# dedis/kyber

Measured on AMD Instinct MI355X. Metric: scalar-muls/s + pairings/s per node; MSM sec at 2^20 points, higher is better.
Workload: dtype int32 limbs (radix 2^25.5), int64 accumulate; 1 GPU; Ed25519 batched fixed-base + var-base scalar-mul, 2^20 scalars per GPU (BASELINE.json configs[1]); elements_per_gpu=1048576

## Files before the change

kyber_amd/csrc/context.h:

```cpp
#pragma once
#include <hip/hip_runtime.h>
#include <stddef.h>
#include <stdint.h>

#include <stdlib.h>
#include <string.h>

#include <algorithm>
#include <condition_variable>
#include <initializer_list>
#include <map>
#include <mutex>
#include <string>
#include <vector>
#include <utility>

#include "../../include/kyber_hip.h"
#include "hd.h"

namespace kyb {

void set_error(const std::string& msg);

#define KYB_HIP_CHECK(expr)                                                              \
    do {                                                                                 \
        hipError_t e_ = (expr);                                                          \
        if (e_ != hipSuccess) {                                                          \
            ::kyb::set_error(std::string(#expr) + ": " + hipGetErrorString(e_));         \
            return KYB_E_HIP;                                                            \
        }                                                                                \
    } while (0)

struct DeviceCtx {
    int device = -1;
    int num_cu = 0;
    bool ready = false;
    std::mutex mu;
    std::recursive_mutex enq_mu;
    int32_t* ed_base_tab = nullptr;
    int32_t* ed_wide_tab = nullptr;
    int64_t ed_wide_build_us = 0;
    struct StreamBuf {
        void* p = nullptr;
        size_t cap = 0;
    };
    std::map<std::pair<int, hipStream_t>, StreamBuf> sws;
    static constexpr int NSTAGE = 12, NPOOL = 2, NPIN = 6;
    struct StagePool {
        bool busy = false;
        hipStream_t stream = nullptr;
        void* stage[NSTAGE] = {};
        size_t stage_cap[NSTAGE] = {};
        hipStream_t pipe[3] = {};
        void* pin_in[NPIN] = {};
        void* pin_out[NPIN] = {};
        bool pinned = false;
    };
    StagePool pools[NPOOL];
    std::mutex stage_mu;
    std::condition_variable stage_cv;
    std::map<std::pair<int, hipStream_t>, std::string> fb_hint;
};
constexpr size_t PIN_SLOT_ELEMS = size_t(1) << 17;
constexpr size_t PIN_IN_BYTES = PIN_SLOT_ELEMS * 64, PIN_OUT_BYTES = PIN_SLOT_ELEMS * 33;
int ctx_pin_slots(DeviceCtx::StagePool* pool);
void par_memcpy(void* dst, const void* src, size_t bytes);

inline int check_flags(uint32_t flags, int npoint, bool point_out, const char* who) {
    const uint32_t allowed = KYB_F_UNCOMPRESSED | (point_out ? KYB_F_UNCOMPRESSED_OUT : 0u) | (((1u << npoint) - 1u) << 8);
    if (flags & ~allowed) {
        set_error(std::string(who) + ": unknown or inapplicable flag bits");
        return KYB_E_ARG;
    }
    return KYB_OK;
}

inline int make_dst(DstArg& d, const uint8_t* dst, size_t dst_len, const char* who) {
    if (dst_len > 255 || (dst_len && !dst)) {
        set_error(std::string(who) + ": the domain separation tag must be at most 255 bytes");
        return KYB_E_ARG;
    }
    memset(&d, 0, sizeof d);
    if (dst_len) memcpy(d.b, dst, dst_len);
    d.len = (uint32_t)dst_len;
    return KYB_OK;
}

int md_count();
size_t md_threshold();
void shard_range(size_t n, int rank, int world, size_t* lo, size_t* hi);
std::vector<int> md_devices();
int md_run_impl(size_t n, int (*thunk)(void*, int, size_t, size_t), void* arg, const std::vector<int>* on = nullptr);
template <class F>
int md_run(size_t n, F&& f, const std::vector<int>* on = nullptr) {
    return md_run_impl(n, [](void* a, int s, size_t lo, size_t hi) -> int { return (*static_cast<F*>(a))(s, lo, hi); }, &f, on);
}
inline bool md_active(size_t n) { return md_count() > 1 && n >= md_threshold() && n >= (size_t)md_count(); }

int get_ctx(DeviceCtx** out);
int ctx_workspace(DeviceCtx* ctx, int kind, hipStream_t stream, size_t bytes, void** out, bool* grew = nullptr);

inline void fb_hint_set(DeviceCtx* ctx, int kind, hipStream_t stream, const std::string* key) {
    std::lock_guard<std::mutex> lk(ctx->mu);
    if (key) ctx->fb_hint[std::make_pair(kind, stream)] = *key;
    else ctx->fb_hint.erase(std::make_pair(kind, stream));
}
inline bool fb_hint_is(DeviceCtx* ctx, int kind, hipStream_t stream, const std::string& key) {
    std::lock_guard<std::mutex> lk(ctx->mu);
    auto it = ctx->fb_hint.find(std::make_pair(kind, stream));
    return it != ctx->fb_hint.end() && it->second == key;
}

struct StageScope {
    DeviceCtx* ctx;
    DeviceCtx::StagePool* pool = nullptr;
    int next = 0;
    explicit StageScope(DeviceCtx* c) : ctx(c) {
        static const int npool = [] {
            const char* e = getenv("KYB_STAGE_POOLS");
            const int v = e ? atoi(e) : 0;
            return v >= 1 && v <= DeviceCtx::NPOOL ? v : DeviceCtx::NPOOL;
        }();
        {
            std::unique_lock<std::mutex> lk(c->stage_mu);
            for (;;) {
                for (int i = 0; i < npool && !pool; i++)
                    if (!c->pools[i].busy) pool = &c->pools[i];
                if (pool) break;
                c->stage_cv.wait(lk);
            }
            pool->busy = true;
        }
        if (!pool->stream && hipStreamCreateWithFlags(&pool->stream, hipStreamDefault) != hipSuccess) pool->stream = nullptr;
        current() = this;
    }
    ~StageScope() {
        current() = nullptr;
        {
            std::lock_guard<std::mutex> lk(ctx->stage_mu);
            pool->busy = false;
        }
        ctx->stage_cv.notify_one();
    }
    StageScope(const StageScope&) = delete;
    StageScope& operator=(const StageScope&) = delete;
    hipStream_t stream() const { return pool->stream; }
    static StageScope*& current() {
        static thread_local StageScope* cur = nullptr;
        return cur;
    }
};
struct StageBuf {
    void* p = nullptr;
    static int too_many() {
        set_error("staging: no scope / too many buffers");
        return KYB_E_ARG;
    }
    int alloc(size_t bytes) {
        StageScope* sc = StageScope::current();
        if (!sc || sc->next >= DeviceCtx::NSTAGE) return too_many();
        const int slot = sc->next++;
        DeviceCtx::StagePool* c = sc->pool;
        if (c->stage_cap[slot] < bytes || !c->stage[slot]) {
            if (c->stage[slot]) {
                hipFree(c->stage[slot]);
                c->stage[slot] = nullptr;
                c->stage_cap[slot] = 0;
            }
            const size_t cap = bytes + bytes / 4 + 256;
            if (hipMalloc(&c->stage[slot], cap) != hipSuccess) {
                set_error("hipMalloc failed");
                return KYB_E_ALLOC;
            }
            c->stage_cap[slot] = cap;
        }
        p = c->stage[slot];
        return KYB_OK;
    }
    static constexpr size_t BOUNCE_MIN = size_t(4) << 20;
    int upload(const void* src, size_t bytes) {
        int rc = alloc(bytes);
        if (rc) return rc;
        if (!bytes) return KYB_OK;
        if (bytes < BOUNCE_MIN) {
            const hipStream_t st = StageScope::current()->stream();
            KYB_HIP_CHECK(hipMemcpyAsync(p, src, bytes, hipMemcpyHostToDevice, st));
            KYB_HIP_CHECK(hipStreamSynchronize(st));
            return KYB_OK;
        }
        return bounce(const_cast<void*>(src), bytes, true);
    }
    int download(void* dst, size_t bytes) {
        if (!bytes) return KYB_OK;
        if (bytes < BOUNCE_MIN) {
            const hipStream_t st = StageScope::current()->stream();
            KYB_HIP_CHECK(hipMemcpyAsync(dst, p, bytes, hipMemcpyDeviceToHost, st));
            KYB_HIP_CHECK(hipStreamSynchronize(st));
            return KYB_OK;
        }
        return bounce(dst, bytes, false);
    }
    int bounce(void* host, size_t bytes, bool up) {
        StageScope* sc = StageScope::current();
        DeviceCtx::StagePool* c = sc->pool;
        const hipStream_t st = sc->stream();
        int rc = ctx_pin_slots(c);
        if (rc) return rc;
        hipEvent_t ev[2];
        for (int k = 0; k < 2; k++) KYB_HIP_CHECK(hipEventCreateWithFlags(&ev[k], hipEventDisableTiming));
        const size_t piece = PIN_IN_BYTES;
        const size_t npiece = (bytes + piece - 1) / piece;
        rc = KYB_OK;
        for (size_t i = 0; i <= npiece && rc == KYB_OK; i++) {
            if (up) {
                if (i == npiece) break;
                const size_t off = i * piece, len = std::min(piece, bytes - off);
                if (i >= 2 && hipEventSynchronize(ev[i & 1]) != hipSuccess) rc = KYB_E_HIP;
                par_memcpy(c->pin_in[i & 1], (const uint8_t*)host + off, len);
                if (hipMemcpyAsync((uint8_t*)p + off, c->pin_in[i & 1], len, hipMemcpyHostToDevice, st) != hipSuccess ||
                    hipEventRecord(ev[i & 1], st) != hipSuccess)
                    rc = KYB_E_HIP;
            } else {
                if (i < npiece) {
                    const size_t off = i * piece, len = std::min(piece, bytes - off);
                    if (hipMemcpyAsync(c->pin_in[i & 1], (const uint8_t*)p + off, len, hipMemcpyDeviceToHost, st) != hipSuccess ||
                        hipEventRecord(ev[i & 1], st) != hipSuccess)
                        rc = KYB_E_HIP;
                }
                if (i >= 1 && rc == KYB_OK) {
                    const size_t off = (i - 1) * piece, len = std::min(piece, bytes - off);
                    if (hipEventSynchronize(ev[(i - 1) & 1]) != hipSuccess) rc = KYB_E_HIP;
                    else par_memcpy((uint8_t*)host + off, c->pin_in[(i - 1) & 1], len);
                }
            }
        }
        if (hipStreamSynchronize(st) != hipSuccess) rc = KYB_E_HIP;
        for (int k = 0; k < 2; k++) hipEventDestroy(ev[k]);
        if (rc == KYB_E_HIP) set_error("staging: page-locked bounce copy failed");
        return rc;
    }
};

struct HostIn {
    const void* p;
    size_t bytes;
    bool absent = false;
};
struct HostOut {
    void* p;
    size_t bytes;
    size_t slack = 0;
};
template <class F>
int staged_call(DeviceCtx* ctx, std::initializer_list<HostIn> in, std::initializer_list<HostOut> out, F&& run) {
    if (in.size() > (size_t)DeviceCtx::NSTAGE || out.size() > (size_t)DeviceCtx::NSTAGE) return StageBuf::too_many();
    StageScope sc(ctx);
    void* d_in[DeviceCtx::NSTAGE] = {};
    void* d_out[DeviceCtx::NSTAGE] = {};
    StageBuf b;
    int k = 0;
    for (const HostIn& h : in) {
        b.p = nullptr;
        if (!h.absent)
            if (int rc = b.upload(h.p, h.bytes)) return rc;
        d_in[k++] = b.p;
    }
    k = 0;
    for (const HostOut& h : out) {
        if (int rc = b.alloc(h.bytes + h.slack)) return rc;
        d_out[k++] = b.p;
    }
    if (int rc = run(d_in, d_out, sc.stream())) return rc;
    k = 0;
    for (const HostOut& h : out) {
        b.p = d_out[k++];
        if (h.p)
            if (int rc = b.download(h.p, h.bytes)) return rc;
    }
    return KYB_OK;
}

int ed25519_build_tables(DeviceCtx* ctx);
void ed25519_free_tables(DeviceCtx* ctx);

}
```

kyber_amd/csrc/ed25519.hip:

```cpp
#ifndef KYB_TU_WAVES
#define KYB_TU_WAVES 2
#endif
#include "context.h"
#include "ed25519_dev.cuh"
#include "ed25519_launch.h"
#include "msm.cuh"
#include "ed25519_h2c.cuh"
#include <stdlib.h>
#include <string.h>

#include <algorithm>
#include <atomic>
#include <chrono>
#include <thread>
#include <vector>

namespace kyb {


template <int G = 2>
__global__ void ed25519_build_base_table_kernel(int32_t* __restrict__ tab, const uint32_t* __restrict__ point,
                                                uint32_t* __restrict__ ok, int rows = ED_TAB_POS * ED_TAB_ENT) {
    const int t = blockIdx.x * blockDim.x + threadIdx.x;
    if (t >= rows) return;
    ge_p3 B;
    if (point) {
        uint32_t pw[8];
        load_words8(pw, point);
        const bool good = ge_p3_fromwords(B, pw);
        if (t == 0) *ok = good ? 1u : 0u;
    } else {
        B.X = fe_bx(); B.Y = fe_by(); fe_1(B.Z); B.T = fe_bt();
    }
    ed_comb_row<G>(tab + (size_t)t * ED_TAB_STRIDE, t, B);
}

__global__ __launch_bounds__(ED_ENC_BLOCK, KYB_TU_WAVES) void ed25519_encode_kernel(size_t n, const int32_t* __restrict__ proj,
                                                            const uint8_t* __restrict__ status,
                                                            uint32_t* __restrict__ out) {
    __shared__ int32_t pre_lds[EncPreLds<ED_ENC_BLOCK>::WORDS];
    static_assert(ED_ENC_BLOCK % 64 == 0 && sizeof(pre_lds) <= 80 * 1024 && sizeof(pre_lds) / (ED_ENC_BLOCK / 64) * 4 <= 160 * 1024,
                  "LDS: at least two blocks on a CU, and a wave on every SIMD");
    EncPreLds<ED_ENC_BLOCK> pre{pre_lds + threadIdx.x};
    ed_encode_chunk(n, proj, ed_encode_first(), blockDim.x, pre, [&](size_t i, uint32_t (&w)[8]) {
        if (status && status[i]) {
#pragma unroll
            for (int k = 0; k < 8; k++) w[k] = 0;
        }
        store_words8(out + i * 8, w);
    });
}


template <int G>
__global__ __launch_bounds__(256, 3) void ed25519_mul_base_kernel(
    size_t n, const uint32_t* __restrict__ scalars, uint32_t* __restrict__ out,
    const int32_t* __restrict__ tab, uint32_t flags, int32_t* __restrict__ proj) {
    const bool full = (flags & KYB_F_VARTIME) != 0;
    for (size_t idx = (size_t)blockIdx.x * blockDim.x + threadIdx.x; idx < n;
         idx += (size_t)gridDim.x * blockDim.x) {
        uint32_t a[8];
        load_words8(a, scalars + idx * 8);
        int8_t e[65];
        recode16(e, a, full);
        ge_p3 h;
        ge_p3_0(h);
        ge_precomp t;
        ge_p1p1 r;
        const int npos = full ? EdComb<G>::POS : EdComb<G>::POS_CT;
        EdCombDigits<G> digits(e);
#pragma unroll 1
        for (int k = 0; k < npos; k++) {
            const int d = digits.next(k);
            if (full && __ballot(d != 0) == 0) continue;
            select_precomp_tab<EdComb<G>::ENT>(t, tab, k, d);
            ge_madd(r, h, t);
            ge_p1p1_to_p3(h, r);
        }
        if (proj) {
            store_proj(proj, idx, h);
            continue;
        }
        uint32_t w[8];
        ge_p3_towords(w, h);
        store_words8(out + idx * 8, w);
    }
}

KYB_DEV void select_precomp_uniform(ge_precomp& t, const int32_t* __restrict__ tab, int i, int b) {
    const bool neg = b < 0;
    const int babs = neg ? -b : b;
    const int pos = i >> 1, mult = (i & 1) ? 16 : 1;
    fe_1(t.ypx);
    fe_1(t.ymx);
    fe_0(t.xy2d);
#pragma unroll 1
    for (int m = 1; m <= 8; m++) {
        const int4* e = reinterpret_cast<const int4*>(tab + (size_t)(pos * ED_TAB_ENT + (m * mult - 1)) * ED_TAB_STRIDE);
        int32_t w[32];
#pragma unroll
        for (int q = 0; q < 8; q++) {
            const int4 x = e[q];
            w[4 * q] = x.x;
            w[4 * q + 1] = x.y;
            w[4 * q + 2] = x.z;
            w[4 * q + 3] = x.w;
        }
        const int32_t keep = -(int32_t)(babs == m);
#pragma unroll
        for (int l = 0; l < 10; l++) {
            t.ypx.v[l] ^= (t.ypx.v[l] ^ w[l]) & keep;
            t.ymx.v[l] ^= (t.ymx.v[l] ^ w[10 + l]) & keep;
            t.xy2d.v[l] ^= (t.xy2d.v[l] ^ w[20 + l]) & keep;
        }
    }
    ge_precomp_cneg(t, neg);
}
__global__ __launch_bounds__(256, 3) void ed25519_mul_base_uniform_kernel(
    size_t n, const uint32_t* __restrict__ scalars, uint32_t* __restrict__ out,
    const int32_t* __restrict__ tab, int32_t* __restrict__ proj) {
    for (size_t idx = (size_t)blockIdx.x * blockDim.x + threadIdx.x; idx < n;
         idx += (size_t)gridDim.x * blockDim.x) {
        uint32_t a[8];
        load_words8(a, scalars + idx * 8);
        int8_t e[65];
        recode16(e, a, false);
        ge_p3 h;
        ge_p3_0(h);
        ge_precomp t;
        ge_p1p1 r;
        EdCombDigits<1> digits(e);
#pragma unroll 1
        for (int i = 0; i < 64; i++) {
            select_precomp_uniform(t, tab, i, digits.next(i));
            ge_madd(r, h, t);
            ge_p1p1_to_p3(h, r);
        }
        if (proj) {
            store_proj(proj, idx, h);
            continue;
        }
        uint32_t w[8];
        ge_p3_towords(w, h);
        store_words8(out + idx * 8, w);
    }
}


template <bool GTAB, bool UNI = false>
__global__ __launch_bounds__(128, 3) void ed25519_mul_kernel(
    size_t n, const uint32_t* __restrict__ scalars, const uint32_t* __restrict__ points,
    size_t points_stride, uint32_t* __restrict__ out, uint8_t* __restrict__ status,
    uint32_t flags, int32_t* __restrict__ proj, int4* __restrict__ gtab) {
    const size_t idx = (size_t)blockIdx.x * blockDim.x + threadIdx.x;
    if (idx >= n) return;
    const bool full = !UNI && (flags & KYB_F_VARTIME) != 0;
    uint32_t pw[8], a[8];
    load_words8(pw, points + idx * points_stride);
    load_words8(a, scalars + idx * 8);
    ge29_p3 A;
    const bool ok = ge_p3_fromwords(A, pw);
    int8_t e[65];
    recode16(e, a, full);
    ge29_p3 h;
    const int vt_top = full ? wave_top_digit(a) : 63;
    if constexpr (GTAB) {
        TabGlobal_t<fe29> tab{gtab + idx * 80};
        ge_scalarmult_w4<UNI, true>(h, e, A, full, tab, vt_top);
    } else {
        TabScratch_t<fe29> tab;
        ge_scalarmult_w4<UNI, true>(h, e, A, full, tab, vt_top);
    }
    if (proj) {
        store_proj(proj, idx, h);
        if (status) status[idx] = ok ? KYB_ST_OK : KYB_ST_BAD_POINT;
        return;
    }
    uint32_t w[8];
    ge_p3_towords(w, h);
    if (!ok) {
#pragma unroll
        for (int i = 0; i < 8; i++) w[i] = 0;
    }
    store_words8(out + idx * 8, w);
    if (status) status[idx] = ok ? KYB_ST_OK : KYB_ST_BAD_POINT;
}

int ed25519_build_tables(DeviceCtx* ctx) {
    KYB_HIP_CHECK(hipMalloc(&ctx->ed_base_tab, ED_TAB_WORDS * sizeof(int32_t)));
    hipLaunchKernelGGL(ed25519_build_base_table_kernel<2>, dim3((ED_TAB_POS * ED_TAB_ENT + 63) / 64), dim3(64), 0,
                       nullptr, ctx->ed_base_tab, (const uint32_t*)nullptr, (uint32_t*)nullptr, ED_TAB_POS * ED_TAB_ENT);
    KYB_HIP_CHECK(hipGetLastError());
    const auto t0 = std::chrono::steady_clock::now();
    KYB_HIP_CHECK(hipMalloc(&ctx->ed_wide_tab, ED_WIDE_WORDS * sizeof(int32_t)));
    hipLaunchKernelGGL(ed25519_build_base_table_kernel<ED_COMB_G>, dim3((EdWide::ROWS + 63) / 64), dim3(64), 0, nullptr,
                       ctx->ed_wide_tab, (const uint32_t*)nullptr, (uint32_t*)nullptr, EdWide::ROWS);
    KYB_HIP_CHECK(hipGetLastError());
    KYB_HIP_CHECK(hipStreamSynchronize(nullptr));
    ctx->ed_wide_build_us = std::chrono::duration_cast<std::chrono::microseconds>(std::chrono::steady_clock::now() - t0).count();
    return KYB_OK;
}
void ed25519_free_tables(DeviceCtx* ctx) {
    if (ctx->ed_base_tab) hipFree(ctx->ed_base_tab);
    if (ctx->ed_wide_tab) hipFree(ctx->ed_wide_tab);
    ctx->ed_base_tab = ctx->ed_wide_tab = nullptr;
}

constexpr size_t ENC_DEFER_MIN = 4096;


static int launch_mul_base(DeviceCtx* ctx, size_t n, const void* d_scalars, void* d_out, uint32_t flags,
                           hipStream_t st, const int32_t* tab = nullptr) {
    const bool wide = !tab && !(flags & KYB_F_UNIFORM);
    if (!tab) tab = wide ? ctx->ed_wide_tab : ctx->ed_base_tab;
    if (n == 0) return KYB_OK;
    const int block = 256;
    size_t want = (n + block - 1) / block;
    size_t cap = (size_t)ctx->num_cu * 8;
    int grid = (int)(want < cap ? want : cap);
    EdSlab w{};
    std::lock_guard<std::recursive_mutex> enq_lock(ctx->enq_mu);
    if (n >= ENC_DEFER_MIN)
        if (int rc = ed_slab(ctx, st, ED_SLAB_MUL_BASE, n, &w)) return rc;
    if (flags & KYB_F_UNIFORM) {
        hipLaunchKernelGGL(ed25519_mul_base_uniform_kernel, dim3(grid), dim3(block), 0, st, n,
                           (const uint32_t*)d_scalars, (uint32_t*)d_out, tab, w.proj);
    } else {
        const auto kernel = wide ? ed25519_mul_base_kernel<ED_COMB_G> : ed25519_mul_base_kernel<2>;
        hipLaunchKernelGGL(kernel, dim3(grid), dim3(block), 0, st, n, (const uint32_t*)d_scalars, (uint32_t*)d_out, tab,
                           flags, w.proj);
    }
    if (w.proj)
        hipLaunchKernelGGL(ed25519_encode_kernel, ed_encode_grid(n), dim3(ED_ENC_BLOCK), 0, st, n, w.proj,
                           (const uint8_t*)nullptr, (uint32_t*)d_out);
    KYB_HIP_CHECK(hipGetLastError());
    return KYB_OK;
}
static int launch_mul(size_t n, const void* d_scalars, const void* d_points, size_t stride, void* d_out,
                      void* d_status, uint32_t flags, hipStream_t st) {
    if (n == 0) return KYB_OK;
    const int block = 128;
    size_t grid = (n + block - 1) / block;
    EdSlab w{};
    uint8_t* stat = (uint8_t*)d_status;
    DeviceCtx* ctx;
    int rc = get_ctx(&ctx);
    if (rc) return rc;
    std::lock_guard<std::recursive_mutex> enq_lock(ctx->enq_mu);
    const bool defer = n >= ENC_DEFER_MIN, uni = (flags & KYB_F_UNIFORM) != 0;
    const auto kernel = defer ? (uni ? ed25519_mul_kernel<true, true> : ed25519_mul_kernel<true, false>)
                              : (uni ? ed25519_mul_kernel<false, true> : ed25519_mul_kernel<false, false>);
    if (defer) {
        if ((rc = ed_slab(ctx, st, ed_slab_mul(stat == nullptr), n, &w))) return rc;
        if (!stat) stat = w.status;
    }
    hipLaunchKernelGGL(kernel, dim3((unsigned)grid), dim3(block), 0, st, n, (const uint32_t*)d_scalars,
                       (const uint32_t*)d_points, stride, (uint32_t*)d_out, stat, flags, w.proj, w.gtab);
    if (w.proj)
        hipLaunchKernelGGL(ed25519_encode_kernel, ed_encode_grid(n), dim3(ED_ENC_BLOCK), 0, st, n, w.proj,
                           (const uint8_t*)stat, (uint32_t*)d_out);
    KYB_HIP_CHECK(hipGetLastError());
    return KYB_OK;
}

}

using namespace kyb;

static bool ed_mul_flags_bad(uint32_t flags) {
    return (flags & ~(KYB_F_VARTIME | KYB_F_UNIFORM)) || (flags & (KYB_F_VARTIME | KYB_F_UNIFORM)) == (KYB_F_VARTIME | KYB_F_UNIFORM);
}

extern "C" {

int kyb_ed25519_mul_base_dev(size_t n, const void* d_scalars, void* d_out, uint32_t flags, void* stream) {
    if ((n && (!d_scalars || !d_out)) || ed_mul_flags_bad(flags)) {
        set_error("kyb_ed25519_mul_base_dev: bad argument");
        return KYB_E_ARG;
    }
    DeviceCtx* ctx;
    int rc = get_ctx(&ctx);
    if (rc) return rc;
    return launch_mul_base(ctx, n, d_scalars, d_out, flags, (hipStream_t)stream);
}

int kyb_ed25519_mul_dev(size_t n, const void* d_scalars, const void* d_points, void* d_out, void* d_status,
                        uint32_t flags, void* stream) {
    if ((n && (!d_scalars || !d_points || !d_out)) || ed_mul_flags_bad(flags)) {
        set_error("kyb_ed25519_mul_dev: bad argument");
        return KYB_E_ARG;
    }
    DeviceCtx* ctx;
    int rc = get_ctx(&ctx);
    if (rc) return rc;
    return launch_mul(n, d_scalars, d_points, 8, d_out, d_status, flags, (hipStream_t)stream);
}

static int mul_host(size_t n, const uint8_t* scalars, const uint8_t* points, size_t stride, uint8_t* out,
                    uint8_t* status, uint32_t flags);

int kyb_ed25519_mul_base(size_t n, const uint8_t* scalars, uint8_t* out, uint32_t flags) {
    if ((n && (!scalars || !out)) || ed_mul_flags_bad(flags)) {
        set_error("kyb_ed25519_mul_base: bad argument");
        return KYB_E_ARG;
    }
    if (n == 0) return KYB_OK;
    if (md_active(n))
        return md_run(n, [&](int, size_t lo, size_t hi) { return kyb_ed25519_mul_base(hi - lo, scalars + 32 * lo, out + 32 * lo, flags); });
    return mul_host(n, scalars, nullptr, 0, out, nullptr, flags);
}

constexpr size_t PIPE_CHUNK_MAX = PIN_SLOT_ELEMS;
constexpr int PIPE_SLOTS = DeviceCtx::NPIN, PIPE_STREAMS = 3;
static size_t pipe_chunk(const DeviceCtx* ctx) {
    if (const char* e = getenv("KYB_PIPE_CHUNK")) {
        const size_t v = (size_t)strtoull(e, nullptr, 10) & ~size_t(63);
        if (v >= 4096) return std::min(PIPE_CHUNK_MAX, v);
    }
    (void)ctx;
    return size_t(1) << 17;
}
static int pipe_nstreams() {
    if (const char* e = getenv("KYB_PIPE_STREAMS")) {
        const int v = atoi(e);
        if (v >= 1 && v <= PIPE_STREAMS) return v;
    }
    return 2;
}
constexpr size_t SAME_BASE_TABLE_MIN = 16384;

static int pipe_streams(DeviceCtx::StagePool* pool) {
    for (int i = 0; i < PIPE_STREAMS; i++)
        if (!pool->pipe[i]) KYB_HIP_CHECK(hipStreamCreateWithFlags(&pool->pipe[i], hipStreamNonBlocking));
    return KYB_OK;
}

static int mul_host(size_t n, const uint8_t* scalars, const uint8_t* points, size_t stride, uint8_t* out,
                    uint8_t* status, uint32_t flags) {
    DeviceCtx* ctx;
    int rc = get_ctx(&ctx);
    if (rc) return rc;
    bool fixed = points == nullptr;
    const size_t npts = fixed ? 0 : (stride ? n : 1);
    StageScope sc_(ctx);
    StageBuf d_s, d_p, d_o, d_st, d_tab;
    if ((rc = d_s.alloc(n * 32))) return rc;
    if ((rc = d_p.alloc(npts * 32))) return rc;
    if ((rc = d_o.alloc(n * 32))) return rc;
    if ((rc = d_st.alloc(n))) return rc;
    const int32_t* tab = nullptr;
    if (!fixed && !stride && (n >= SAME_BASE_TABLE_MIN || (flags & KYB_F_UNIFORM))) {
        if ((rc = d_tab.alloc(ED_TAB_WORDS * sizeof(int32_t) + 256))) return rc;
        uint32_t* d_ok = (uint32_t*)((uint8_t*)d_tab.p + ED_TAB_WORDS * sizeof(int32_t));
        KYB_HIP_CHECK(hipMemcpy(d_p.p, points, 32, hipMemcpyHostToDevice));
        hipLaunchKernelGGL(ed25519_build_base_table_kernel<2>, dim3((ED_TAB_POS * ED_TAB_ENT + 63) / 64), dim3(64), 0, sc_.stream(),
                           (int32_t*)d_tab.p, (const uint32_t*)d_p.p, d_ok, ED_TAB_POS * ED_TAB_ENT);
        uint32_t ok = 0;
        KYB_HIP_CHECK(hipMemcpy(&ok, d_ok, 4, hipMemcpyDeviceToHost));
        if (!ok) {
            memset(out, 0, n * 32);
            if (status) memset(status, KYB_ST_BAD_POINT, n);
            return KYB_OK;
        }
        if (status) memset(status, 0, n);
        tab = (const int32_t*)d_tab.p;
        fixed = true;
    }
    auto launch = [&](size_t off, size_t cnt, hipStream_t st) -> int {
        uint8_t* s = (uint8_t*)d_s.p + off * 32;
        uint8_t* o = (uint8_t*)d_o.p + off * 32;
        if (fixed) return launch_mul_base(ctx, cnt, s, o, flags, st, tab);
        const uint8_t* p = (const uint8_t*)d_p.p + (stride ? off * 32 : 0);
        return launch_mul(cnt, s, p, stride, o, (uint8_t*)d_st.p + off, flags, st);
    };
    const size_t PIPE_CHUNK = pipe_chunk(ctx);
    if (n < 2 * PIPE_CHUNK) {
        KYB_HIP_CHECK(hipMemcpy(d_s.p, scalars, n * 32, hipMemcpyHostToDevice));
        if (npts) KYB_HIP_CHECK(hipMemcpy(d_p.p, points, npts * 32, hipMemcpyHostToDevice));
        if ((rc = launch(0, n, nullptr))) return rc;
        if ((rc = d_o.download(out, n * 32))) return rc;
        if (status && !fixed) rc = d_st.download(status, n);
        return rc;
    }
    DeviceCtx::StagePool* pool = sc_.pool;
    if ((rc = pipe_streams(pool))) return rc;
    const int nstreams = pipe_nstreams();
    const bool per_point = !fixed && stride;
    const bool want_status = status && !fixed;
    if ((rc = ctx_pin_slots(pool))) return rc;
    const size_t nchunks = (n + PIPE_CHUNK - 1) / PIPE_CHUNK;
    std::vector<hipEvent_t> ev_out(nchunks);
    for (size_t i = 0; i < nchunks; i++) KYB_HIP_CHECK(hipEventCreateWithFlags(&ev_out[i], hipEventDisableTiming));
    auto enqueue = [&](size_t i) -> int {
        const size_t off = i * PIPE_CHUNK, cnt = std::min(PIPE_CHUNK, n - off);
        uint8_t* pin = (uint8_t*)pool->pin_in[i % PIPE_SLOTS];
        uint8_t* pout = (uint8_t*)pool->pin_out[i % PIPE_SLOTS];
        hipStream_t s_k = pool->pipe[i % nstreams];
        par_memcpy(pin, scalars + off * 32, cnt * 32);
        if (per_point) par_memcpy(pin + PIPE_CHUNK_MAX * 32, points + off * 32, cnt * 32);
        int r;
        if (fixed) {
            r = launch_mul_base(ctx, cnt, pin, pout, flags, s_k, tab);
        } else {
            const uint8_t* p = per_point ? pin + PIPE_CHUNK_MAX * 32 : (const uint8_t*)d_p.p;
            r = launch_mul(cnt, pin, p, stride, pout, (uint8_t*)d_st.p + off, flags, s_k);
        }
        if (r) return r;
        if (want_status)
            KYB_HIP_CHECK(hipMemcpyAsync(pout + PIPE_CHUNK_MAX * 32, (uint8_t*)d_st.p + off, cnt, hipMemcpyDeviceToHost, s_k));
        KYB_HIP_CHECK(hipEventRecord(ev_out[i], s_k));
        return KYB_OK;
    };
    auto drain = [&](size_t i) -> int {
        const size_t off = i * PIPE_CHUNK, cnt = std::min(PIPE_CHUNK, n - off);
        KYB_HIP_CHECK(hipEventSynchronize(ev_out[i]));
        const uint8_t* pout = (const uint8_t*)pool->pin_out[i % PIPE_SLOTS];
        par_memcpy(out + off * 32, pout, cnt * 32);
        if (want_status) memcpy(status + off, pout + PIPE_CHUNK_MAX * 32, cnt);
        return KYB_OK;
    };
    if (!fixed && !stride) KYB_HIP_CHECK(hipMemcpy(d_p.p, points, 32, hipMemcpyHostToDevice));
    std::atomic<size_t> enqueued{0}, drained{0};
    std::atomic<int> drain_rc{KYB_OK};
    std::atomic<bool> stop{false};
    const int device = ctx->device;
    std::string drain_err;
    std::thread drainer([&] {
        if (hipSetDevice(device) != hipSuccess) {
            drain_err = "ed25519 host pipeline: hipSetDevice failed on the drain thread";
            drain_rc.store(KYB_E_HIP);
            return;
        }
        for (size_t i = 0; i < nchunks; i++) {
            while (enqueued.load(std::memory_order_acquire) <= i) {
                if (stop.load(std::memory_order_acquire)) return;
                std::this_thread::yield();
            }
            const int r = drain(i);
            if (r) {
                drain_err = kyb_last_error();
                drain_rc.store(r);
                return;
            }
            drained.store(i + 1, std::memory_order_release);
        }
    });
    for (size_t i = 0; i < nchunks && rc == KYB_OK; i++) {
        while (i >= (size_t)PIPE_SLOTS && drained.load(std::memory_order_acquire) + PIPE_SLOTS <= i && drain_rc.load() == KYB_OK)
            std::this_thread::yield();
        if (drain_rc.load() != KYB_OK) break;
        rc = enqueue(i);
        if (rc == KYB_OK) enqueued.store(i + 1, std::memory_order_release);
    }
    if (rc != KYB_OK) stop.store(true, std::memory_order_release);
    drainer.join();
    if (rc == KYB_OK && (rc = drain_rc.load()) != KYB_OK) set_error(drain_err);
    hipError_t e2 = hipSuccess;
    for (int i = 0; i < PIPE_STREAMS; i++) {
        const hipError_t e = hipStreamSynchronize(pool->pipe[i]);
        if (e != hipSuccess) e2 = e;
    }
    for (size_t i = 0; i < nchunks; i++) hipEventDestroy(ev_out[i]);
    if (rc == KYB_OK && e2 != hipSuccess) {
        set_error("ed25519 host pipeline: stream synchronisation failed");
        rc = KYB_E_HIP;
    }
    return rc;
}

int kyb_ed25519_mul(size_t n, const uint8_t* scalars, const uint8_t* points, uint8_t* out, uint8_t* status,
                    uint32_t flags) {
    if ((n && (!scalars || !points || !out)) || ed_mul_flags_bad(flags)) {
        set_error("kyb_ed25519_mul: bad argument");
        return KYB_E_ARG;
    }
    if (n == 0) return KYB_OK;
    if (md_active(n))
        return md_run(n, [&](int, size_t lo, size_t hi) {
            return kyb_ed25519_mul(hi - lo, scalars + 32 * lo, points + 32 * lo, out + 32 * lo, status ? status + lo : nullptr, flags);
        });
    return mul_host(n, scalars, points, 8, out, status, flags);
}

int kyb_ed25519_mul_same_base(size_t n, const uint8_t* scalars, const uint8_t point[32], uint8_t* out,
                              uint8_t* status, uint32_t flags) {
    if ((n && (!scalars || !out)) || !point || ed_mul_flags_bad(flags)) {
        set_error("kyb_ed25519_mul_same_base: bad argument");
        return KYB_E_ARG;
    }
    if (n == 0) return KYB_OK;
    if (md_active(n))
        return md_run(n, [&](int, size_t lo, size_t hi) {
            return kyb_ed25519_mul_same_base(hi - lo, scalars + 32 * lo, point, out + 32 * lo, status ? status + lo : nullptr, flags);
        });
    return mul_host(n, scalars, point, 0, out, status, flags);
}

int kyb_ed25519_debug_base_table(int32_t* out) {
    if (!out) return KYB_E_ARG;
    DeviceCtx* ctx;
    int rc = get_ctx(&ctx);
    if (rc) return rc;
    KYB_HIP_CHECK(hipMemcpy(out, ctx->ed_base_tab, ED_TAB_WORDS * sizeof(int32_t), hipMemcpyDeviceToHost));
    return KYB_OK;
}

int kyb_ed25519_comb_info(int64_t info[6]) {
    if (!info) return KYB_E_ARG;
    DeviceCtx* ctx;
    int rc = get_ctx(&ctx);
    if (rc) return rc;
    info[0] = ED_COMB_G;
    info[1] = EdWide::POS;
    info[2] = EdWide::ENT;
    info[3] = EdWide::LAST_ENT;
    info[4] = (int64_t)(ED_WIDE_WORDS * sizeof(int32_t));
    info[5] = ctx->ed_wide_build_us;
// ... 274 lines not shown
```

kyber_amd/csrc/ed25519_dev.cuh:

```cuda
#pragma once
#include "ge25519.cuh"

#if !defined(__HIPCC__)
#include <type_traits>
struct int4 { int32_t x, y, z, w; };
struct uint4 { uint32_t x, y, z, w; };
inline int4 make_int4(int32_t x, int32_t y, int32_t z, int32_t w) { return int4{x, y, z, w}; }
inline uint4 make_uint4(uint32_t x, uint32_t y, uint32_t z, uint32_t w) { return uint4{x, y, z, w}; }
#define KYB_DEV_CONST static
#else
#define KYB_DEV_CONST __device__
#endif

namespace kyb {

constexpr int ED_TAB_POS = 33;
constexpr int ED_TAB_ENT = 136;
constexpr int ED_TAB_STRIDE = 32;
constexpr int ED_TAB_WORDS = ED_TAB_POS * ED_TAB_ENT * ED_TAB_STRIDE;

template <int G>
struct EdComb {
    static constexpr int POS = (65 + G - 1) / G;
    static constexpr int POS_CT = (64 + G - 1) / G;
    static constexpr int ENT = 8 * ((1 << (4 * G)) - 1) / 15;
    static constexpr int LAST_D = 65 - G * (POS - 1);
    static constexpr int LAST_ENT = 8 * ((1 << (4 * LAST_D)) - 1) / 15;
    static constexpr int ROWS = (POS - 1) * ENT + LAST_ENT;
};
#ifndef ED_COMB_G
#define ED_COMB_G 4
#endif
using EdWide = EdComb<ED_COMB_G>;
constexpr size_t ED_WIDE_WORDS = (size_t)EdWide::ROWS * ED_TAB_STRIDE;

KYB_DEV void load_words8(uint32_t w[8], const uint32_t* __restrict__ p) {
    const uint4 a = reinterpret_cast<const uint4*>(p)[0];
    const uint4 b = reinterpret_cast<const uint4*>(p)[1];
    w[0] = a.x; w[1] = a.y; w[2] = a.z; w[3] = a.w;
    w[4] = b.x; w[5] = b.y; w[6] = b.z; w[7] = b.w;
}
KYB_DEV void store_words8(uint32_t* __restrict__ p, const uint32_t w[8]) {
    reinterpret_cast<uint4*>(p)[0] = make_uint4(w[0], w[1], w[2], w[3]);
    reinterpret_cast<uint4*>(p)[1] = make_uint4(w[4], w[5], w[6], w[7]);
}

template <int G>
KYB_DEV void ed_comb_row(int32_t* __restrict__ o, int t, const ge_p3& B) {
    constexpr int ENT = EdComb<G>::ENT;
    const int pos = t / ENT, j = t - pos * ENT;
    ge_cached cB;
    ge_p3_to_cached(cB, B);
    ge_p3 acc;
    ge_p3_0(acc);
    ge_p1p1 r;
#pragma unroll 1
    for (int bit = 4 * G - 1; bit >= 0; bit--) {
        ge_dbl(r, acc.X, acc.Y, acc.Z);
        ge_p1p1_to_p3(acc, r);
        if (((j + 1) >> bit) & 1) {
            ge_add(r, acc, cB);
            ge_p1p1_to_p3(acc, r);
        }
    }
#pragma unroll 1
    for (int k = 0; k < 4 * G * pos; k++) {
        ge_dbl(r, acc.X, acc.Y, acc.Z);
        ge_p1p1_to_p3(acc, r);
    }
    fe zi, x, y, ypx, ymx, xy2d, z;
    fe_invert(zi, acc.Z);
    fe_mul(x, acc.X, zi);
    fe_mul(y, acc.Y, zi);
    fe_add(ypx, y, x);
    fe_sub(ymx, y, x);
    fe_mul(xy2d, x, y);
    fe_mul(xy2d, xy2d, fe_d2());
    fe_1(z);
    fe_mul(ypx, ypx, z);
    fe_mul(ymx, ymx, z);
#pragma unroll
    for (int l = 0; l < 10; l++) {
        o[l] = ypx.v[l];
        o[10 + l] = ymx.v[l];
        o[20 + l] = xy2d.v[l];
    }
    o[30] = o[31] = 0;
}

constexpr int ENC_CHUNK = 16;

KYB_DEV void store_proj(int32_t* __restrict__ proj, size_t idx, const ge_p3& h) {
    int32_t* o = proj + idx * 30;
#pragma unroll
    for (int l = 0; l < 10; l++) {
        o[l] = h.X.v[l];
        o[10 + l] = h.Y.v[l];
        o[20 + l] = h.Z.v[l];
    }
}
KYB_DEV void store_proj(int32_t* __restrict__ proj, size_t idx, const ge29_p3& h) {
    ge_p3 t;
    fe29_to_fe(t.X, h.X);
    fe29_to_fe(t.Y, h.Y);
    fe29_to_fe(t.Z, h.Z);
    store_proj(proj, idx, t);
}
KYB_DEV void load_fe(fe& f, const int32_t* __restrict__ p) {
#pragma unroll
    for (int l = 0; l < 10; l++) f.v[l] = p[l];
}
struct EncPreScratch {
    fe pre[ENC_CHUNK];
    KYB_DEV void put(int j, const fe& f) { pre[j] = f; }
    KYB_DEV void get(fe& f, int j) const { f = pre[j]; }
};
template <int LANES>
struct EncPreLds {
    int32_t* col;
    static constexpr int WORDS = ENC_CHUNK * 10 * LANES;
    KYB_DEV void put(int j, const fe& f) {
#pragma unroll
        for (int l = 0; l < 10; l++) col[(j * 10 + l) * LANES] = f.v[l];
    }
    KYB_DEV void get(fe& f, int j) const {
#pragma unroll
        for (int l = 0; l < 10; l++) f.v[l] = col[(j * 10 + l) * LANES];
        KYB_FE_MAG_SET(f, 1.01);
    }
};
#if defined(__HIPCC__)
template <int GROUP = 1>
KYB_DEV size_t ed_encode_first() {
    return (size_t)blockIdx.x * blockDim.x * (ENC_CHUNK / GROUP) + threadIdx.x;
}
#endif
template <int GROUP = 1, class Pre, class Emit>
KYB_DEV void ed_encode_chunk(size_t n, const int32_t* __restrict__ proj, size_t first, size_t stride, Pre& pre, Emit emit) {
    static_assert(GROUP >= 1 && GROUP <= ENC_CHUNK, "whole records per lane");
    int cnt = 0;
#pragma unroll
    for (int r = 0; r < ENC_CHUNK / GROUP; r++) cnt += (first + r * stride < n) ? GROUP : 0;
    if (cnt == 0) return;
    auto point = [&](int j) { return (first + (size_t)(j / GROUP) * stride) * GROUP + (size_t)(j % GROUP); };
    fe z, acc;
    load_fe(acc, proj + point(0) * 30 + 20);
    pre.put(0, acc);
#pragma unroll 1
    for (int j = 1; j < cnt; j++) {
        load_fe(z, proj + point(j) * 30 + 20);
        fe_mul(acc, acc, z);
        pre.put(j, acc);
    }
    fe inv;
    fe_invert(inv, acc);
#pragma unroll 1
    for (int j = cnt - 1; j >= 0; j--) {
        const size_t i = point(j);
        fe zi, X, Y;
        load_fe(z, proj + i * 30 + 20);
        if (j > 0) {
            pre.get(zi, j - 1);
            fe_mul(zi, inv, zi);
            fe_mul(inv, inv, z);
        } else {
            zi = inv;
        }
        load_fe(X, proj + i * 30);
        load_fe(Y, proj + i * 30 + 10);
        uint32_t w[8];
        ge_encode_with_zinv(w, X, Y, zi);
        emit(i, w);
    }
}

template <int ENT>
KYB_DEV void select_precomp_tab(ge_precomp& t, const int32_t* __restrict__ tab, int pos, int b) {
    const bool neg = b < 0;
    const int babs = neg ? -b : b;
    const int4* e = reinterpret_cast<const int4*>(tab + (size_t)(pos * ENT + (babs ? babs - 1 : 0)) * ED_TAB_STRIDE);
    int32_t w[32];
#pragma unroll
    for (int i = 0; i < 8; i++) {
        const int4 x = e[i];
        w[4 * i] = x.x;
        w[4 * i + 1] = x.y;
        w[4 * i + 2] = x.z;
        w[4 * i + 3] = x.w;
    }
#pragma unroll
    for (int l = 0; l < 10; l++) {
        t.ypx.v[l] = w[l];
        t.ymx.v[l] = w[10 + l];
        t.xy2d.v[l] = w[20 + l];
    }
    if (babs == 0) {
        fe_1(t.ypx);
        fe_1(t.ymx);
        fe_0(t.xy2d);
    }
    ge_precomp_cneg(t, neg);
}

KYB_DEV void ed_pack_digits(uint32_t pk[8], const int8_t e[65]) {
#pragma unroll
    for (int j = 0; j < 8; j++) {
        pk[j] = 0;
#pragma unroll
        for (int q = 0; q < 8; q++) pk[j] |= (uint32_t)((e[8 * j + q] + 8) & 15) << (4 * q);
    }
}

template <int G>
struct EdCombDigits {
    static_assert(G >= 1 && G <= 7, "a position's digits are read from one 32-bit word");
    static constexpr int PACKED = 63 / G;
    static constexpr int TAIL = EdComb<G>::POS - PACKED;
    uint32_t pk[8];
    int tail[TAIL];
    KYB_DEV explicit EdCombDigits(const int8_t e[65]) {
        ed_pack_digits(pk, e);
#pragma unroll
        for (int t = 0; t < TAIL; t++) {
            int d = 0;
#pragma unroll
            for (int i = G - 1; i >= 0; i--)
                if (G * (PACKED + t) + i <= 64) d = 16 * d + (int)e[G * (PACKED + t) + i];
            tail[t] = d;
        }
    }
    KYB_DEV int next(int k) {
        int d = (int)(pk[0] & ((1u << (4 * G)) - 1u)) - EdComb<G>::ENT;
#pragma unroll
        for (int j = 0; j < 7; j++) pk[j] = (pk[j] >> (4 * G)) | (pk[j + 1] << (32 - 4 * G));
        pk[7] >>= 4 * G;
#pragma unroll
        for (int t = 0; t < TAIL; t++)
            if (k == PACKED + t) d = tail[t];
        return d;
    }
};

template <class F = fe>
struct TabScratch_t {
    typedef typename ge_t<F>::cached cached;
    cached tab[8];
    KYB_DEV void put(int j, const cached& c) { tab[j] = c; }
    KYB_DEV void get(cached& c, int j) const { c = tab[j]; }
};
using TabScratch = TabScratch_t<>;
template <class F = fe>
struct TabGlobal_t;
using TabGlobal = TabGlobal_t<>;
template <>
struct TabGlobal_t<fe> {
    int4* base;
    KYB_DEV void put(int j, const ge_cached& c) {
        int4* q = base + j * 10;
        const fe* f[4] = {&c.YpX, &c.YmX, &c.Z, &c.T2d};
        int32_t w[40];
#pragma unroll
        for (int k = 0; k < 4; k++)
#pragma unroll
            for (int l = 0; l < 10; l++) w[10 * k + l] = f[k]->v[l];
#pragma unroll
        for (int i = 0; i < 10; i++) q[i] = make_int4(w[4 * i], w[4 * i + 1], w[4 * i + 2], w[4 * i + 3]);
    }
    KYB_DEV void get(ge_cached& c, int j) const {
        const int4* q = base + j * 10;
        int32_t w[40];
#pragma unroll
        for (int i = 0; i < 10; i++) {
            const int4 x = q[i];
            w[4 * i] = x.x;
            w[4 * i + 1] = x.y;
            w[4 * i + 2] = x.z;
            w[4 * i + 3] = x.w;
        }
        fe* f[4] = {&c.YpX, &c.YmX, &c.Z, &c.T2d};
#pragma unroll
        for (int k = 0; k < 4; k++)
#pragma unroll
            for (int l = 0; l < 10; l++) f[k]->v[l] = w[10 * k + l];
    }
    KYB_DEV void get_signed(ge_cached& c, int b) const;
};
KYB_DEV_CONST __attribute__((aligned(16))) const int32_t ED_CACHED_IDENTITY[40] = {1, 0, 0, 0, 0, 0, 0, 0, 0, 0,
                                                                               1, 0, 0, 0, 0, 0, 0, 0, 0, 0,
                                                                               1};
KYB_DEV void TabGlobal_t<fe>::get_signed(ge_cached& c, int b) const {
    const bool neg = b < 0;
    const int babs = neg ? -b : b;
#if defined(__HIPCC__)
    typedef int32_t i32x2 __attribute__((ext_vector_type(2)));
    typedef int32_t i32x4 __attribute__((ext_vector_type(4)));
    using gint = const __attribute__((address_space(1))) int32_t;
    using gint2 = const __attribute__((address_space(1))) i32x2;
    using gint4 = const __attribute__((address_space(1))) i32x4;
#else
    struct i32x2 { int32_t x, y; };
    struct i32x4 { int32_t x, y, z, w; };
    using gint = const int32_t;
    using gint2 = const i32x2;
    using gint4 = const i32x4;
#endif
    gint* e = babs ? (gint*)(base + (babs - 1) * 10) : (gint*)ED_CACHED_IDENTITY;
    gint2* p = (gint2*)(e + (neg ? 10 : 0));
    gint2* m = (gint2*)(e + (neg ? 0 : 10));
    gint4* q = (gint4*)(e + 20);
#pragma unroll
    for (int i = 0; i < 5; i++) {
        const i32x2 x = p[i], y = m[i];
        c.YpX.v[2 * i] = x.x;
        c.YpX.v[2 * i + 1] = x.y;
        c.YmX.v[2 * i] = y.x;
        c.YmX.v[2 * i + 1] = y.y;
    }
    int32_t w[20];
#pragma unroll
    for (int i = 0; i < 5; i++) {
        const i32x4 x = q[i];
        w[4 * i] = x.x;
        w[4 * i + 1] = x.y;
        w[4 * i + 2] = x.z;
        w[4 * i + 3] = x.w;
    }
    const int32_t s = -(int32_t)neg;
#pragma unroll
    for (int l = 0; l < 10; l++) {
        c.Z.v[l] = w[l];
        c.T2d.v[l] = (w[10 + l] ^ s) - s;
    }
}
template <>
struct TabGlobal_t<fe29> {
    int4* base;
    static constexpr int word(int field, int l) { return field < 2 ? (l < 8 ? 8 * field + l : 16 + field) : 18 + 9 * (field - 2) + l; }
    KYB_DEV void put(int j, const ge29_cached& c) {
        int4* q = base + j * 9;
        const fe29* f[4] = {&c.YpX, &c.YmX, &c.Z, &c.T2d};
        int32_t w[36];
#pragma unroll
        for (int k = 0; k < 4; k++)
#pragma unroll
            for (int l = 0; l < 9; l++) w[word(k, l)] = f[k]->v[l];
#pragma unroll
        for (int i = 0; i < 9; i++) q[i] = make_int4(w[4 * i], w[4 * i + 1], w[4 * i + 2], w[4 * i + 3]);
    }
    KYB_DEV void get(ge29_cached& c, int j) const {
        const int4* q = base + j * 9;
        int32_t w[36];
#pragma unroll
        for (int i = 0; i < 9; i++) {
            const int4 x = q[i];
            w[4 * i] = x.x;
            w[4 * i + 1] = x.y;
            w[4 * i + 2] = x.z;
            w[4 * i + 3] = x.w;
        }
        fe29* f[4] = {&c.YpX, &c.YmX, &c.Z, &c.T2d};
#pragma unroll
        for (int k = 0; k < 4; k++)
#pragma unroll
            for (int l = 0; l < 9; l++) f[k]->v[l] = w[word(k, l)];
        KYB_FE_MAG_SET(c.YpX, 3.001);
        KYB_FE_MAG_SET(c.YmX, 3.001);
        KYB_FE_MAG_SET(c.Z, 1.001);
        KYB_FE_MAG_SET(c.T2d, 1.001);
    }
    KYB_DEV void get_signed(ge29_cached& c, int b) const;
};
KYB_DEV_CONST __attribute__((aligned(16))) const int32_t ED_CACHED_IDENTITY29[36] = {1, 0, 0, 0, 0, 0, 0, 0,
                                                                                 1, 0, 0, 0, 0, 0, 0, 0,
                                                                                 0, 0, 1};
KYB_DEV void TabGlobal_t<fe29>::get_signed(ge29_cached& c, int b) const {
    const bool neg = b < 0;
    const int babs = neg ? -b : b;
#if defined(__HIPCC__)
    typedef int32_t i32x4 __attribute__((ext_vector_type(4)));
    using gint = const __attribute__((address_space(1))) int32_t;
    using gint4 = const __attribute__((address_space(1))) i32x4;
#else
    struct i32x4 { int32_t x, y, z, w; };
    using gint = const int32_t;
    using gint4 = const i32x4;
#endif
    gint* e = babs ? (gint*)(base + (babs - 1) * 9) : (gint*)ED_CACHED_IDENTITY29;
    gint4* p = (gint4*)(e + (neg ? 8 : 0));
    gint4* m = (gint4*)(e + (neg ? 0 : 8));
    gint4* q = (gint4*)(e + 16);
#pragma unroll
    for (int i = 0; i < 2; i++) {
        const i32x4 x = p[i], y = m[i];
        c.YpX.v[4 * i] = x.x;
        c.YpX.v[4 * i + 1] = x.y;
        c.YpX.v[4 * i + 2] = x.z;
        c.YpX.v[4 * i + 3] = x.w;
        c.YmX.v[4 * i] = y.x;
        c.YmX.v[4 * i + 1] = y.y;
        c.YmX.v[4 * i + 2] = y.z;
        c.YmX.v[4 * i + 3] = y.w;
    }
    int32_t w[20];
#pragma unroll
    for (int i = 0; i < 5; i++) {
        const i32x4 x = q[i];
        w[4 * i] = x.x;
        w[4 * i + 1] = x.y;
        w[4 * i + 2] = x.z;
        w[4 * i + 3] = x.w;
    }
    c.YpX.v[8] = neg ? w[1] : w[0];
    c.YmX.v[8] = neg ? w[0] : w[1];
    const int32_t s = -(int32_t)neg;
#pragma unroll
    for (int l = 0; l < 9; l++) {
        c.Z.v[l] = w[2 + l];
        c.T2d.v[l] = (w[11 + l] ^ s) - s;
    }
    KYB_FE_MAG_SET(c.YpX, 3.001);
    KYB_FE_MAG_SET(c.YmX, 3.001);
    KYB_FE_MAG_SET(c.Z, 1.001);
    KYB_FE_MAG_SET(c.T2d, 1.001);
}
template <bool UNI = false, class C, class Tab>
KYB_DEV void select_cached(C& c, const Tab& tab, int b) {
    typedef decltype(c.Z) F;
    const bool neg = b < 0;
    const int babs = neg ? -b : b;
    if constexpr (UNI) {
        ge_cached_0(c);
#pragma unroll 1
        for (int m = 1; m <= 8; m++) {
            C x;
            tab.get(x, m - 1);
            const int32_t keep = -(int32_t)(babs == m);
#pragma unroll
            for (int l = 0; l < F::N; l++) {
                c.YpX.v[l] ^= (c.YpX.v[l] ^ x.YpX.v[l]) & keep;
                c.YmX.v[l] ^= (c.YmX.v[l] ^ x.YmX.v[l]) & keep;
                c.Z.v[l] ^= (c.Z.v[l] ^ x.Z.v[l]) & keep;
                c.T2d.v[l] ^= (c.T2d.v[l] ^ x.T2d.v[l]) & keep;
            }
        }
    } else if constexpr (std::is_same_v<Tab, TabGlobal_t<F>>) {
        tab.get_signed(c, b);
        return;
    } else {
        tab.get(c, babs ? babs - 1 : 0);
        if (babs == 0) ge_cached_0(c);
    }
    ge_cached_cneg(c, neg);
}

KYB_DEV int wave_top_digit(const uint32_t a[8]) {
    int bits = 0;
#pragma unroll
    for (int i = 0; i < 8; i++)
        if (a[i]) bits = 32 * i + 32 - __builtin_clz(a[i]);
    int t = (bits + 3) >> 2;
    if (t > 64) t = 64;
#if defined(__HIP_DEVICE_COMPILE__)
#pragma unroll
    for (int off = 32; off >= 1; off >>= 1) {
        const int o = __shfl_xor(t, off, 64);
        t = o > t ? o : t;
    }
    t = __builtin_amdgcn_readfirstlane(t);
#endif
    return t;
}

template <bool AFFINE = false, class P3, class Tab>
KYB_DEV void ge_window_table(Tab& tab, const P3& A) {
    typedef ge_t<decltype(A.X)> G;
    typename G::p1p1 t;
    P3 u;
    typename G::cached c;
    ge_p3_to_cached(c, A);
    tab.put(0, c);
    if constexpr (AFFINE) {
        const typename G::precomp a{c.YpX, c.YmX, c.T2d};
        u = A;
#pragma unroll 1
        for (int i = 0; i < 7; i++) {
            ge_madd(t, u, a);
            ge_p1p1_to_p3(u, t);
            ge_p3_to_cached(c, u);
            tab.put(i + 1, c);
        }
    } else {
#pragma unroll 1
        for (int i = 0; i < 7; i++) {
            ge_add(t, A, c);
            ge_p1p1_to_p3(u, t);
            ge_p3_to_cached(c, u);
            tab.put(i + 1, c);
        }
    }
}

template <bool UNI = false, bool AFFINE = false, class P3, class Tab>
KYB_DEV void ge_scalarmult_w4(P3& h, const int8_t e[65], const P3& A, bool full, Tab& tab, int vt_top) {
    typedef ge_t<decltype(A.X)> G;
    typename G::p1p1 t;
    P3 u;
    typename G::p2 r;
    typename G::cached c;
    ge_window_table<AFFINE>(tab, A);
    ge_p3_0(u);
    int top = 63;
    if (full) top = vt_top;
    select_cached<UNI>(c, tab, e[top]);
    ge_add(t, u, c);
    uint32_t pk[8];
    ed_pack_digits(pk, e);
    auto shl4 = [&pk]() {
#pragma unroll
        for (int j = 7; j > 0; j--) pk[j] = (pk[j] << 4) | (pk[j - 1] >> 28);
        pk[0] <<= 4;
    };
#pragma unroll 1
    for (int i = top; i < 64; i++) shl4();
#pragma unroll 1
    for (int i = top - 1; i >= 0; i--) {
        const int d = (int)(pk[7] >> 28) - 8;
        shl4();
        ge_p1p1_to_p2(r, t);
        ge_dbl(t, r.X, r.Y, r.Z);
        ge_p1p1_to_p2(r, t);
        ge_dbl(t, r.X, r.Y, r.Z);
        ge_p1p1_to_p2(r, t);
        ge_dbl(t, r.X, r.Y, r.Z);
        ge_p1p1_to_p2(r, t);
        ge_dbl(t, r.X, r.Y, r.Z);
#if defined(__HIP_DEVICE_COMPILE__)
        if (!UNI && full && __ballot(d != 0) == 0) continue;
#endif
        ge_p1p1_to_p3(u, t);
        select_cached<UNI>(c, tab, d);
        ge_add(t, u, c);
    }
    ge_p1p1_to_p3(h, t);
}
// ... 3 lines not shown
```

Before: 197.5 million scalar-muls/s.

## Store wide comb table in nine-limb fe29 form and walk it in fe29

Adds a second wide fixed-base table in a 9-limb radix-2^29 representation, with a zero-digit identity row appended, and switches the wide fixed-base comb walk to fe29 arithmetic for G>2. The aim is cheaper field multiplies in the madd loop, fewer limbs to load per table entry, and a branch-free identity and negation select. The cost is extra device memory for a second table and a longer table build.

Result: no change. 198.5 million scalar-muls/s, median of 6 (+0.5%).

```diff
diff --git a/kyber_amd/csrc/context.h b/kyber_amd/csrc/context.h
--- a/kyber_amd/csrc/context.h
+++ b/kyber_amd/csrc/context.h
@@ -40,6 +40,7 @@
     int32_t* ed_base_tab = nullptr;
     int32_t* ed_wide_tab = nullptr;
     int64_t ed_wide_build_us = 0;
+    int32_t* ed_wide_tab29 = nullptr;
     struct StreamBuf {
         void* p = nullptr;
         size_t cap = 0;
diff --git a/kyber_amd/csrc/ed25519.hip b/kyber_amd/csrc/ed25519.hip
--- a/kyber_amd/csrc/ed25519.hip
+++ b/kyber_amd/csrc/ed25519.hip
@@ -20,8 +20,10 @@
 
 template <int G = 2>
 __global__ void ed25519_build_base_table_kernel(int32_t* __restrict__ tab, const uint32_t* __restrict__ point,
-                                                uint32_t* __restrict__ ok, int rows = ED_TAB_POS * ED_TAB_ENT) {
+                                                uint32_t* __restrict__ ok, int rows = ED_TAB_POS * ED_TAB_ENT,
+                                                int32_t* __restrict__ tab29 = nullptr) {
     const int t = blockIdx.x * blockDim.x + threadIdx.x;
+    if (t == rows && tab29) ed_comb_identity29(tab29 + (size_t)t * ED_TAB_STRIDE);
     if (t >= rows) return;
     ge_p3 B;
     if (point) {
@@ -32,7 +34,7 @@
     } else {
         B.X = fe_bx(); B.Y = fe_by(); fe_1(B.Z); B.T = fe_bt();
     }
-    ed_comb_row<G>(tab + (size_t)t * ED_TAB_STRIDE, t, B);
+    ed_comb_row<G>(tab + (size_t)t * ED_TAB_STRIDE, t, B, tab29 ? tab29 + (size_t)t * ED_TAB_STRIDE : nullptr);
 }
 
 __global__ __launch_bounds__(ED_ENC_BLOCK, KYB_TU_WAVES) void ed25519_encode_kernel(size_t n, const int32_t* __restrict__ proj,
@@ -63,20 +65,8 @@
         load_words8(a, scalars + idx * 8);
         int8_t e[65];
         recode16(e, a, full);
-        ge_p3 h;
-        ge_p3_0(h);
-        ge_precomp t;
-        ge_p1p1 r;
-        const int npos = full ? EdComb<G>::POS : EdComb<G>::POS_CT;
-        EdCombDigits<G> digits(e);
-#pragma unroll 1
-        for (int k = 0; k < npos; k++) {
-            const int d = digits.next(k);
-            if (full && __ballot(d != 0) == 0) continue;
-            select_precomp_tab<EdComb<G>::ENT>(t, tab, k, d);
-            ge_madd(r, h, t);
-            ge_p1p1_to_p3(h, r);
-        }
+        typename ge_t<EdCombField<G>>::p3 h;
+        ed_comb_walk<G>(h, e, full, tab);
         if (proj) {
             store_proj(proj, idx, h);
             continue;
@@ -193,8 +183,9 @@
     KYB_HIP_CHECK(hipGetLastError());
     const auto t0 = std::chrono::steady_clock::now();
     KYB_HIP_CHECK(hipMalloc(&ctx->ed_wide_tab, ED_WIDE_WORDS * sizeof(int32_t)));
-    hipLaunchKernelGGL(ed25519_build_base_table_kernel<ED_COMB_G>, dim3((EdWide::ROWS + 63) / 64), dim3(64), 0, nullptr,
-                       ctx->ed_wide_tab, (const uint32_t*)nullptr, (uint32_t*)nullptr, EdWide::ROWS);
+    KYB_HIP_CHECK(hipMalloc(&ctx->ed_wide_tab29, ED_WIDE29_WORDS * sizeof(int32_t)));
+    hipLaunchKernelGGL(ed25519_build_base_table_kernel<ED_COMB_G>, dim3((EdWide::ROWS + 1 + 63) / 64), dim3(64), 0, nullptr,
+                       ctx->ed_wide_tab, (const uint32_t*)nullptr, (uint32_t*)nullptr, EdWide::ROWS, ctx->ed_wide_tab29);
     KYB_HIP_CHECK(hipGetLastError());
     KYB_HIP_CHECK(hipStreamSynchronize(nullptr));
     ctx->ed_wide_build_us = std::chrono::duration_cast<std::chrono::microseconds>(std::chrono::steady_clock::now() - t0).count();
@@ -203,7 +194,8 @@
 void ed25519_free_tables(DeviceCtx* ctx) {
     if (ctx->ed_base_tab) hipFree(ctx->ed_base_tab);
     if (ctx->ed_wide_tab) hipFree(ctx->ed_wide_tab);
-    ctx->ed_base_tab = ctx->ed_wide_tab = nullptr;
+    if (ctx->ed_wide_tab29) hipFree(ctx->ed_wide_tab29);
+    ctx->ed_base_tab = ctx->ed_wide_tab = ctx->ed_wide_tab29 = nullptr;
 }
 
 constexpr size_t ENC_DEFER_MIN = 4096;
@@ -212,7 +204,7 @@
 static int launch_mul_base(DeviceCtx* ctx, size_t n, const void* d_scalars, void* d_out, uint32_t flags,
                            hipStream_t st, const int32_t* tab = nullptr) {
     const bool wide = !tab && !(flags & KYB_F_UNIFORM);
-    if (!tab) tab = wide ? ctx->ed_wide_tab : ctx->ed_base_tab;
+    if (!tab) tab = wide ? ctx->ed_wide_tab29 : ctx->ed_base_tab;
     if (n == 0) return KYB_OK;
     const int block = 256;
     size_t want = (n + block - 1) / block;
diff --git a/kyber_amd/csrc/ed25519_dev.cuh b/kyber_amd/csrc/ed25519_dev.cuh
--- a/kyber_amd/csrc/ed25519_dev.cuh
+++ b/kyber_amd/csrc/ed25519_dev.cuh
@@ -45,8 +45,35 @@
     reinterpret_cast<uint4*>(p)[1] = make_uint4(w[4], w[5], w[6], w[7]);
 }
 
+constexpr size_t ED_WIDE29_WORDS = ((size_t)EdWide::ROWS + 1) * ED_TAB_STRIDE;
+constexpr int ed_row29_word(int field, int l) { return field < 2 ? (l < 8 ? 8 * field + l : 16 + field) : 18 + l; }
+
+KYB_DEV void ed_comb_row29(int32_t* __restrict__ o, const fe& ypx, const fe& ymx, const fe& xy2d) {
+    const fe* f[3] = {&ypx, &ymx, &xy2d};
+#pragma unroll
+    for (int k = 0; k < 3; k++) {
+        fe29 h;
+        fe29_from_fe(h, *f[k]);
+#pragma unroll
+        for (int i = 0; i < 8; i++) {
+            const int32_t c = (h.v[i] + (1 << 28)) >> 29;
+            h.v[i] -= c * (1 << 29);
+            h.v[i + 1] += c;
+        }
+#pragma unroll
+        for (int l = 0; l < 9; l++) o[ed_row29_word(k, l)] = h.v[l];
+    }
+#pragma unroll
+    for (int l = 27; l < ED_TAB_STRIDE; l++) o[l] = 0;
+}
+KYB_DEV void ed_comb_identity29(int32_t* __restrict__ o) {
+#pragma unroll
+    for (int l = 0; l < ED_TAB_STRIDE; l++) o[l] = 0;
+    o[ed_row29_word(0, 0)] = o[ed_row29_word(1, 0)] = 1;
+}
+
 template <int G>
-KYB_DEV void ed_comb_row(int32_t* __restrict__ o, int t, const ge_p3& B) {
+KYB_DEV void ed_comb_row(int32_t* __restrict__ o, int t, const ge_p3& B, int32_t* __restrict__ o29 = nullptr) {
     constexpr int ENT = EdComb<G>::ENT;
     const int pos = t / ENT, j = t - pos * ENT;
     ge_cached cB;
@@ -86,6 +113,7 @@
         o[20 + l] = xy2d.v[l];
     }
     o[30] = o[31] = 0;
+    if (o29) ed_comb_row29(o29, ypx, ymx, xy2d);
 }
 
 constexpr int ENC_CHUNK = 16;
@@ -201,6 +229,54 @@
     }
     ge_precomp_cneg(t, neg);
 }
+template <int ENT>
+KYB_DEV void select_precomp_tab(ge29_precomp& t, const int32_t* __restrict__ tab, int pos, int b) {
+    static_assert(ENT == EdWide::ENT, "the nine-limb table is the wide comb's");
+    const bool neg = b < 0;
+    const int babs = neg ? -b : b;
+#if defined(__HIPCC__)
+    typedef int32_t i32x4 __attribute__((ext_vector_type(4)));
+    using gint = const __attribute__((address_space(1))) int32_t;
+    using gint4 = const __attribute__((address_space(1))) i32x4;
+#else
+    struct i32x4 { int32_t x, y, z, w; };
+    using gint = const int32_t;
+    using gint4 = const i32x4;
+#endif
+    gint* e = (gint*)(tab + (size_t)(babs ? pos * ENT + babs - 1 : EdWide::ROWS) * ED_TAB_STRIDE);
+    gint4* p = (gint4*)(e + (neg ? 8 : 0));
+    gint4* m = (gint4*)(e + (neg ? 0 : 8));
+    gint4* q = (gint4*)(e + 16);
+#pragma unroll
+    for (int i = 0; i < 2; i++) {
+        const i32x4 x = p[i], y = m[i];
+        t.ypx.v[4 * i] = x.x;
+        t.ypx.v[4 * i + 1] = x.y;
+        t.ypx.v[4 * i + 2] = x.z;
+        t.ypx.v[4 * i + 3] = x.w;
+        t.ymx.v[4 * i] = y.x;
+        t.ymx.v[4 * i + 1] = y.y;
+        t.ymx.v[4 * i + 2] = y.z;
+        t.ymx.v[4 * i + 3] = y.w;
+    }
+    int32_t w[12];
+#pragma unroll
+    for (int i = 0; i < 3; i++) {
+        const i32x4 x = q[i];
+        w[4 * i] = x.x;
+        w[4 * i + 1] = x.y;
+        w[4 * i + 2] = x.z;
+        w[4 * i + 3] = x.w;
+    }
+    t.ypx.v[8] = neg ? w[1] : w[0];
+    t.ymx.v[8] = neg ? w[0] : w[1];
+    const int32_t s = -(int32_t)neg;
+#pragma unroll
+    for (int l = 0; l < 9; l++) t.xy2d.v[l] = (w[2 + l] ^ s) - s;
+    KYB_FE_MAG_SET(t.ypx, 1.001);
+    KYB_FE_MAG_SET(t.ymx, 1.001);
+    KYB_FE_MAG_SET(t.xy2d, 1.001);
+}
 
 KYB_DEV void ed_pack_digits(uint32_t pk[8], const int8_t e[65]) {
 #pragma unroll
@@ -240,6 +316,31 @@
         return d;
     }
 };
+
+template <int G>
+using EdCombField = std::conditional_t<(G > 2), fe29, fe>;
+template <int G>
+KYB_DEV void ed_comb_walk(typename ge_t<EdCombField<G>>::p3& h, const int8_t e[65], bool full,
+                          const int32_t* __restrict__ tab) {
+    typedef ge_t<EdCombField<G>> T;
+    typename T::p3 acc;
+    ge_p3_0(acc);
+    typename T::precomp t;
+    typename T::p1p1 r;
+    const int npos = full ? EdComb<G>::POS : EdComb<G>::POS_CT;
+    EdCombDigits<G> digits(e);
+#pragma unroll 1
+    for (int k = 0; k < npos; k++) {
+        const int d = digits.next(k);
+#if defined(__HIP_DEVICE_COMPILE__)
+        if (full && __ballot(d != 0) == 0) continue;
+#endif
+        select_precomp_tab<EdComb<G>::ENT>(t, tab, k, d);
+        ge_madd(r, acc, t);
+        ge_p1p1_to_p3(acc, r);
+    }
+    h = acc;
+}
 
 template <class F = fe>
 struct TabScratch_t {
```
